# ShuhongChen/panic3d-anime-reconstruction

Hardware: AMD Instinct MI355X
Metric: rendered rays/sec at 512^2 img x 96 samples/ray (higher is better)
Workload: dtype f32

## Files before the change

### panic3d-anime-reconstruction_amd/csrc/p3d_kernels.hip

```cpp
#include <hip/hip_runtime.h>
#include <stddef.h>
#include <stdlib.h>
#include <string.h>

#include <atomic>
#include <type_traits>

#include "p3d_ray_phases.hpp"
#include "p3d_render_plan.hpp"
#include "p3d_cull_band.hpp"
#include "p3d_phase_timing.hpp"

#define P3D_WAVES_PER_WG 4
#define P3D_WG (64 * P3D_WAVES_PER_WG)

__global__ __launch_bounds__(256) void k_planes_to_nhwc(const float* __restrict__ src, float* __restrict__ dst, int HW) {
    __shared__ float tile[32][65];
    const int p0 = blockIdx.x * 64;
    const size_t img = (size_t)blockIdx.y * 32 * HW;
    {
        int px = threadIdx.x & 63, c0 = threadIdx.x >> 6;
#pragma unroll
        for (int k = 0; k < 8; ++k) {
            int c = c0 + 4 * k;
// ... 210 lines not shown
    if (tile >= p.ntiles) return;
    P3D_PHASE(P3D_PH_WEIGHTS);
    float* wl = lds + (FAST ? P3D_LDS_FAST_FLOATS : P3D_LDS_MLP_FLOATS) + 4 + (size_t)wave * p.lds_rows * 32;
    const int Sc = p.Sc, Sf = P3D_NF_EXACT(NF) ? NF : p.Sf, S = Sc + Sf;
    const P3dRayCtx cx = p3d_ray_setup(p, p3d_render_tile_ray(p, tile, j), Sc, Sf);
    const bool active = cx.active;
    const size_t ray = cx.ray;
    const float ox = cx.ox, oy = cx.oy, oz = cx.oz, dx = cx.dx, dy = cx.dy, dz = cx.dz;
    constexpr bool early = EARLY;
    int ndec = 0;

    float* tcA = wl;
    float* wcA = TCG ? wl : tcA + Sc * 32;
    float* tfA = (NF > 0) ? wcA : wcA + Sc * 32;
    uint32_t* mkA = (uint32_t*)(wl + (size_t)(p.lds_rows - ((Sc + 31) >> 5)) * 32);
    const int nmw = (S + 31) >> 5;
    uint32_t* knA = TCG ? (uint32_t*)(wl + (size_t)(Sc > Sf ? Sc : Sf) * 32) : mkA - (size_t)2 * nmw * 32;
    uint32_t* slA = knA + (size_t)nmw * 32;
    const P3dSpacing sp = TCG ? p3d_spacing_fixed(p.ray_start, p.ray_end, p.depth_delta, Sc) : p3d_spacing_of(p, ray, Sc);
    auto tc_raw = [&](int i) -> float { return p3d_stratified_fixed(i, Sc, cx.jitter(i), sp); };
    auto tc_of = [&](int i) -> float { if constexpr (TCG) return tc_raw(i); else return tcA[i * 32 + j]; };
    bool wave_unsorted = false;
    bool bad_order = false;
    bool wave_bad = false;
    auto tc_sorted = [&](int i) -> float { return p3d_coarse_rank(tc_raw, i, Sc, wave_unsorted, wave_bad); };
    uint32_t mw0 = 0u, mw1 = 0u, mw2 = 0u;
    uint32_t fw0 = 0u, fw1 = 0u, fw2 = 0u;
    const bool dump = DUMP && active && h == 0;

    bool unsorted = false;
    float tcmin = __builtin_inff(), tcmax = -__builtin_inff();
    if constexpr (!TCG) {
        float prev = -__builtin_inff();
        for (int i0 = 0; i0 < Sc; i0 += 8) {
            float jv[8];
#pragma unroll
            for (int q = 0; q < 8; ++q) jv[q] = cx.jitter(i0 + q < Sc ? i0 + q : Sc - 1);
#pragma unroll
            for (int q = 0; q < 8; ++q) {
                const int i = i0 + q;
                if (i < Sc) {
                    const float t = p3d_stratified_depth(i, Sc, jv[q], sp);
                    tcA[i * 32 + j] = t;
                    unsorted |= (t < prev);
                    prev = t;
                    tcmin = __builtin_fminf(tcmin, t);
                    tcmax = __builtin_fmaxf(tcmax, t);
                    if constexpr (DUMP) if (dump && p.dumps.depths_coarse) p.dumps.depths_coarse[ray * Sc + i] = t;
                }
            }
        }
    }
    P3D_PHASE(P3D_PH_STRAT);
    float tmin = __builtin_inff(), tmax = -__builtin_inff();
    if (Sf > 0) {
        MarchState st = p3d_march_start();
        uint32_t mword = 0;
        if constexpr (TCG) {
            float prev = -__builtin_inff(), pmax = -__builtin_inff();
            for (int i0 = 0; i0 < Sc; i0 += 8) {
                float jv[8];
#pragma unroll
                for (int q = 0; q < 8; ++q) jv[q] = cx.jitter(i0 + q < Sc ? i0 + q : Sc - 1);
#pragma unroll
                for (int q = 0; q < 8; ++q) {
                    const int i = i0 + q;
                    if (i >= Sc) break;
                    const float t = p3d_stratified_fixed(i, Sc, jv[q], sp);
                    unsorted |= (t < prev);
                    bad_order |= (t < pmax);
                    pmax = __builtin_fmaxf(pmax, prev);
                    prev = t;
                    tcmin = __builtin_fminf(tcmin, t);
                    tcmax = __builtin_fmaxf(tcmax, t);
                    const float px = ox + t * dx, py = oy + t * dy, pz = oz + t * dz;
                    float sigma = P3D_SIGMA_MASKED;
                    const bool cropped = cx.cropped(px, pz);
                    const bool live = !(cropped || st.Td < 1e-60);
                    const bool skip = __builtin_amdgcn_ballot_w64(live) == 0;
                    if (!skip) {
                        f32x16 dummy;
                        p3d_decode_wave<false, true>(lds, cx.rs, cx.g, cx.cfg, px, py, pz, sigma, dummy, live);
                    }
                    mword |= (cropped || (live && sigma == P3D_SIGMA_MASKED)) ? (1u << (i & 31)) : 0u;
                    if ((i & 31) == 31 || i == Sc - 1) {
                        if ((i >> 5) == 0) mw0 = mword; else if ((i >> 5) == 1) mw1 = mword; else mw2 = mword;
                        mword = 0;
                    }
                    if (i > 0) wcA[(i - 1) * 32 + j] = p3d_march_interval(st, t, sigma).w;
                    st.prev_t = t; st.prev_sigma = sigma;
                    ndec += skip ? 0 : 1;
                }
            }
        } else
        for (int i = 0; i < Sc; ++i) {
            float t = tcA[i * 32 + j];
            float px = ox + t * dx, py = oy + t * dy, pz = oz + t * dz;
            float sigma = P3D_SIGMA_MASKED;
            bool skip = false, live = true, cropped = false;
            if (early) {
                cropped = cx.cropped(px, pz);
                live = !(cropped || st.Td < 1e-60);
                skip = __builtin_amdgcn_ballot_w64(live) == 0;
            }
            if (!skip) {
                f32x16 dummy;
                p3d_decode_wave<false, true>(lds, cx.rs, cx.g, cx.cfg, px, py, pz, sigma, dummy, live);
            }
            if (early) {
                mword |= (cropped || (live && sigma == P3D_SIGMA_MASKED)) ? (1u << (i & 31)) : 0u;
                if ((i & 31) == 31 || i == Sc - 1) { mkA[(i >> 5) * 32 + j] = mword; mword = 0; }
            }
            if constexpr (DUMP) if (dump && p.dumps.sigma_coarse) p.dumps.sigma_coarse[ray * Sc + i] = sigma;
            if (i > 0) {
                float w = p3d_march_interval(st, t, sigma).w;
                wcA[(i - 1) * 32 + j] = w;
                if constexpr (DUMP) if (dump && p.dumps.weights_coarse) p.dumps.weights_coarse[ray * (Sc - 1) + i - 1] = w;
            }
            st.prev_t = t; st.prev_sigma = sigma;
            if constexpr (!DUMP) ndec += skip ? 0 : 1;
        }
        P3D_PHASE(P3D_PH_COARSE);
        const int Ns = Sc - 3;
        p3d_pdf_to_cdf<32>(wcA, Ns, j);
        P3D_PHASE(P3D_PH_CDF);
        constexpr int DB = P3D_DRAW_BATCH;
        auto dump_draw = [&](bool mine, int i, float v, int k) {
            if constexpr (DUMP) {
                if (mine && p.dumps.depths_fine) p.dumps.depths_fine[ray * Sf + i] = v;
                if (mine && p.dumps.inds) p.dumps.inds[ray * Sf + i] = k;
            }
        };
        if constexpr (P3D_NF_EXACT(NF)) {
            constexpr int H = NF / 2;
            static_assert(H % DB == 0, "whole batches of draws per half");
            const int d0 = h * H;
            float tf[H];
#pragma unroll
            for (int i = 0; i < H; ++i) tf[i] = cx.u(d0 + i);
#pragma unroll
            for (int i0 = 0; i0 < H; i0 += DB) {
                float ub[DB], vb[DB];
                int kb[DB];
#pragma unroll
                for (int q = 0; q < DB; ++q) ub[q] = tf[i0 + q];
                p3d_inverse_cdf<DB, 32>(wcA, tc_of, Ns, j, ub, vb, kb);
#pragma unroll
                for (int q = 0; q < DB; ++q) {
                    tf[i0 + q] = vb[q];
                    dump_draw(active, d0 + i0 + q, vb[q], kb[q]);
                }
            }
            P3D_PHASE(P3D_PH_DRAWS);
// ... 40 lines not shown
            P3D_PHASE(P3D_PH_DRAWS);
            p3d_sort_network<NF>(tf);
#pragma unroll
            for (int i = 0; i < NF; ++i)
                if (i < Sf) {
                    tfA[i * 32 + j] = tf[i];
                    if constexpr (TCG) {
                        const uint32_t b = cx.cropped_at(tf[i]) ? (1u << (i & 31)) : 0u;
                        if (i < 32) fw0 |= b; else if (i < 64) fw1 |= b; else fw2 |= b;
                    }
                }
        } else {
            for (int i0 = 0; i0 < Sf; i0 += DB) {
                float ub[DB], vb[DB];
                int kb[DB];
#pragma unroll
                for (int q = 0; q < DB; ++q) ub[q] = cx.u(i0 + q < Sf ? i0 + q : Sf - 1);
                p3d_inverse_cdf<DB, 32>(wcA, tc_of, Ns, j, ub, vb, kb);
#pragma unroll
                for (int q = 0; q < DB; ++q) {
                    if (i0 + q < Sf) {
                        tfA[(i0 + q) * 32 + j] = vb[q];
                        dump_draw(dump, i0 + q, vb[q], kb[q]);
                    }
                }
            }
            P3D_PHASE(P3D_PH_DRAWS);
            p3d_lds_insertion_sort(tfA, Sf, j);
        }
        P3D_PHASE(P3D_PH_SORT);
        if constexpr (TCG) {
            wave_unsorted = __builtin_amdgcn_ballot_w64(unsorted) != 0;
            wave_bad = __builtin_amdgcn_ballot_w64(bad_order) != 0;
            if (wave_unsorted) { mw0 = 0u; mw1 = 0u; mw2 = 0u; }
        } else
        if (__builtin_amdgcn_ballot_w64(unsorted) != 0) {
            p3d_lds_insertion_sort(tcA, Sc, j);
            if (early) {
                for (int i = 0; i < ((Sc + 31) >> 5); ++i) mkA[i * 32 + j] = 0u;
            }
        }
    }
    MarchState st = p3d_march_start();
    P3dAccum acc;
    f32x16 prev_rgb = 0.0f;
    {
        int ci = 0, fi = 0;
        float ta = TCG ? 0.0f : tcA[j], tb = (Sf > 0) ? tfA[j] : __builtin_inff();
        tmin = __builtin_fminf(tcmin, tb);
        tmax = __builtin_fmaxf(tcmax, (Sf > 0) ? tfA[(Sf - 1) * 32 + j] : -__builtin_inff());
        bool prev_skipped = false, first = true, done = false;
        int m = 0;
        auto advance = [&](bool take_c) {
            ci += take_c ? 1 : 0;
            fi += take_c ? 0 : 1;
            const int cq = ci < Sc ? ci : Sc - 1, fq = fi < Sf ? fi : (Sf > 0 ? Sf - 1 : 0);
            const float nv = (take_c ? tcA : tfA)[(take_c ? cq : fq) * 32 + j];
            ta = take_c ? nv : ta;
            tb = take_c ? tb : nv;
        };
        float tcn = 0.0f;
        if constexpr (TCG) {
            p3d_merge_bits_ranks(
                tc_sorted, [&](int k) { return tfA[k * 32 + j]; },
                [&](int i, float t) {
                    const uint32_t mwv = (i < 32) ? mw0 : (i < 64 ? mw1 : mw2);
                    return cx.cropped_at(t) || ((mwv >> (i & 31)) & 1u);
                },
                [&](int w, uint32_t kw, uint32_t sw) { knA[w * 32 + j] = kw; slA[w * 32 + j] = sw; }, fw0, fw1, fw2, Sc, Sf, h);
            tcn = tc_sorted(0);
        } else
        if constexpr (EARLY) {
            for (int w = 0; w < nmw; ++w) { knA[w * 32 + j] = 0u; slA[w * 32 + j] = 0u; }
            __builtin_amdgcn_fence(__ATOMIC_ACQ_REL, "wavefront");
            p3d_merge_bits_half(
                [&](bool c, int i) { return (c ? tcA : tfA)[i * 32 + j]; },
                [&](bool c, int i, float t) {
                    bool known = cx.cropped_at(t);
                    if (c && Sf > 0) known = known || ((mkA[(i >> 5) * 32 + j] >> (i & 31)) & 1u);
                    return known;
                },
                [&](int w, uint32_t kw, uint32_t sw) { atomicOr(&knA[w * 32 + j], kw); atomicOr(&slA[w * 32 + j], sw); },
                Sc, Sf, h);
            __builtin_amdgcn_fence(__ATOMIC_ACQ_REL, "wavefront");
            ci = 0;
        }
        P3D_PHASE(P3D_PH_MERGE);
        for (int it = 0;; ++it) {
            bool take_c, known = false;
            float t;
            if constexpr (!EARLY) {
                if (it >= S) break;
                take_c = (ci < Sc) && (fi >= Sf || ta <= tb);
                t = take_c ? ta : tb;
                advance(take_c);
            } else {
                if (!done && (m >= S || st.Td < (FAST ? P3D_FAST_TD_CUT : 1e-60))) done = true;
                if (!done && (first || st.prev_sigma <= 602.0f)) {
                    bool any = false, last_c = false;
                    while (m < S) {
                        const int sh = m & 31, left = (32 - sh < S - m) ? 32 - sh : S - m;
                        const uint32_t kw = knA[(m >> 5) * 32 + j] >> sh, sw = slA[(m >> 5) * 32 + j] >> sh;
                        int run = (~kw != 0u) ? __builtin_ctz(~kw) : 32;
                        run = run < left ? run : left;
                        if (run > 0) {
                            const uint32_t inrun = run >= 32 ? 0xffffffffu : ((1u << run) - 1u);
                            ci += __builtin_popcount(sw & inrun);
                            last_c = (sw >> (run - 1)) & 1u;
                            any = true;
                            m += run;
                        }
                        if (run < left) break;
                    }
// ... 604 lines not shown
                            int force_sigmoid, float* out_sigma, float* out_rgb, void* stream) {
    if (!feats || !w0 || !b0 || !w1 || !b1 || !out_sigma || !out_rgb || N <= 0 || M <= 0) return P3D_E_ARG;
    if ((((uintptr_t)feats | (uintptr_t)out_rgb) & 15) != 0) return P3D_E_RANGE;
    DecodeFeatParams p;
    p.feats = feats; p.w0 = w0; p.b0 = b0; p.w1 = w1; p.b1 = b1; p.out_sigma = out_sigma; p.out_rgb = out_rgb;
    p.M = M; p.tiles_per_img = (M + 31) / 32; p.ntiles = p.tiles_per_img * N;
    memset(&p.cfg, 0, sizeof(p.cfg));
    p.cfg.flags = force_sigmoid ? P3D_FLAG_FORCE_SIGMOID : 0;
    const size_t lds_bytes = (size_t)(P3D_LDS_MLP_FLOATS + 4) * 4;
    long long blocks = (p.ntiles + P3D_WAVES_PER_WG - 1) / P3D_WAVES_PER_WG;
    if (blocks > 256 * 8) blocks = 256 * 8;
    hipError_t e = p3d_ensure_dynamic_lds(k_decode_features, lds_bytes);
    if (e != hipSuccess) return (int)e;
    hipLaunchKernelGGL(k_decode_features, dim3((unsigned)blocks), dim3(P3D_WG), lds_bytes, (hipStream_t)stream, p);
    return p3d_check_launch();
}

size_t p3d_render_workspace_bytes(int N, int64_t R, int Sc, int Sf) {
    (void)R; (void)Sc; (void)Sf;
    return p3d_render_plan_workspace_bytes(N);
}

#ifdef P3D_PHASE_TIMING
int p3d_phase_read(unsigned long long* out, int n, int reset) {
    unsigned long long v[P3D_PH_N];
    if (hipDeviceSynchronize() != hipSuccess || hipMemcpyFromSymbol(v, HIP_SYMBOL(g_p3d_phase), sizeof(v)) != hipSuccess) return -1;
    for (int q = 0; q < n && q < P3D_PH_N; ++q) out[q] = v[q];
    if (reset) {
        memset(v, 0, sizeof(v));
        if (hipMemcpyToSymbol(HIP_SYMBOL(g_p3d_phase), v, sizeof(v)) != hipSuccess) return -1;
    }
    return P3D_PH_N;
}
#endif
int p3d_render_plan_info(int N, int64_t R, int ray_tile_w, const p3d_opts* opts, int has_dumps, int has_ray_limits, int64_t* out, int cap) {
    if (!opts) return P3D_E_ARG;
    const RenderPlan pl = p3d_render_plan(N, R, ray_tile_w, *opts, has_dumps != 0, has_ray_limits != 0);
    if (pl.err) return pl.err;
    if (!out || cap < 6) return P3D_E_ARG;
    const int64_t info[6] = {pl.slots, pl.ntiles, pl.decode_steps_full, pl.grid, pl.block, (int64_t)pl.lds_bytes};
    for (int i = 0; i < 6; ++i) out[i] = info[i];
    return P3D_OK;
}

int p3d_render_f32(const float* planes, int N, int H, int W, const float* rays_o, const float* rays_d, int64_t R,
                   int ray_tile_w, const float* jitter, const float* u, const float* w0, const float* b0,
                   const float* w1, const float* b1, const p3d_opts* opts, float* out_feat, float* out_depth,
                   float* out_wsum, float* out_xyz, void* workspace, size_t workspace_bytes, const p3d_dumps* dumps,
                   void* stream) {
    return p3d_render_limits_f32(planes, N, H, W, rays_o, rays_d, R, ray_tile_w, jitter, u, w0, b0, w1, b1, nullptr, nullptr, opts,
                                 out_feat, out_depth, out_wsum, out_xyz, workspace, workspace_bytes, dumps, stream);
}

static int render_impl(const float* planes, int N, int H, int W, const float* rays_o, const float* rays_d, int64_t R,
                       int ray_tile_w, const float* jitter, const float* u, int rng, uint64_t seed, const float* w0, const float* b0,
                       const float* w1, const float* b1, const float* ray_start, const float* ray_end, const p3d_opts* opts,
                       float* out_feat, float* out_depth, float* out_wsum, float* out_xyz, void* workspace,
                       size_t workspace_bytes, const p3d_dumps* dumps, void* stream);

int p3d_render_limits_f32(const float* planes, int N, int H, int W, const float* rays_o, const float* rays_d, int64_t R,
                          int ray_tile_w, const float* jitter, const float* u, const float* w0, const float* b0,
                          const float* w1, const float* b1, const float* ray_start, const float* ray_end, const p3d_opts* opts,
                          float* out_feat, float* out_depth, float* out_wsum, float* out_xyz, void* workspace,
                          size_t workspace_bytes, const p3d_dumps* dumps, void* stream) {
    return render_impl(planes, N, H, W, rays_o, rays_d, R, ray_tile_w, jitter, u, 0, 0, w0, b0, w1, b1, ray_start, ray_end, opts, out_feat,
                       out_depth, out_wsum, out_xyz, workspace, workspace_bytes, dumps, stream);
// ... 9 lines not shown

static int render_impl(const float* planes, int N, int H, int W, const float* rays_o, const float* rays_d, int64_t R,
                       int ray_tile_w, const float* jitter, const float* u, int rng, uint64_t seed, const float* w0, const float* b0,
                       const float* w1, const float* b1, const float* ray_start, const float* ray_end, const p3d_opts* opts,
                       float* out_feat, float* out_depth, float* out_wsum, float* out_xyz, void* workspace,
                       size_t workspace_bytes, const p3d_dumps* dumps, void* stream) {
    if ((ray_start == nullptr) != (ray_end == nullptr)) return P3D_E_ARG;
    if (!planes || !rays_o || !rays_d || (!jitter && !rng) || !w0 || !b0 || !w1 || !b1 || !opts || !out_feat || !out_depth ||
        !out_wsum || !out_xyz || !workspace || N <= 0 || R <= 0)
        return P3D_E_ARG;
    const int Sc = opts->Sc, Sf = opts->Sf;
    if (Sc < 4 || Sc > P3D_MAX_S || Sf < 0 || Sf > P3D_MAX_S) return P3D_E_RANGE;
    if (Sf > 0 && !u && !rng) return P3D_E_ARG;
    if (H <= 0 || W <= 0 || (long long)H * W * 128 * 3 >= 0x7ffffff0LL) return P3D_E_RANGE;
    if (workspace_bytes < p3d_render_plan_workspace_bytes(N)) return P3D_E_WORKSPACE;
    const RenderPlan pl = p3d_render_plan(N, R, ray_tile_w, *opts, dumps != nullptr, ray_start != nullptr);
    if (pl.err) return pl.err;
    hipStream_t st = (hipStream_t)stream;
    RenderParams p;
    p.planes = planes; p.rays_o = rays_o; p.rays_d = rays_d; p.jitter = jitter; p.u = u;
    p.rng = rng; p.seed_lo = (uint32_t)seed; p.seed_hi = (uint32_t)(seed >> 32);
    p.w0 = w0; p.b0 = b0; p.w1 = w1; p.b1 = b1;
    p.out_feat = out_feat; p.out_depth = out_depth; p.out_wsum = out_wsum; p.out_xyz = out_xyz;
    p.gminmax = (uint32_t*)workspace;
    p.per_view_clamp = (opts->flags & P3D_FLAG_PER_VIEW_CLAMP) ? 1 : 0;
    if (dumps) p.dumps = *dumps; else memset(&p.dumps, 0, sizeof(p.dumps));
    p.R = R; p.H = H; p.W = W; p.Sc = Sc; p.Sf = Sf;
    p.ray_start = opts->ray_start; p.ray_end = opts->ray_end; p.depth_delta = opts->depth_delta;
    p.ray_start_arr = ray_start; p.ray_end_arr = ray_end;
    p.disparity = (opts->flags & P3D_FLAG_DISPARITY) ? 1 : 0;
    p.white_back = (opts->flags & P3D_FLAG_WHITE_BACK) ? 1 : 0;
    p.cfg = make_cfg(opts);
    p.tile_w = pl.tile_w; p.tiles_x = pl.tiles_x; p.tiles_per_img = pl.tiles_per_img; p.ntiles = pl.ntiles;
    p.lds_rows = pl.lds_rows; p.swz = pl.swz; p.blocked = pl.blocked;
    hipLaunchKernelGGL(k_minmax_init, dim3((unsigned)((N + 255) / 256)), dim3(256), 0, st, p.gminmax, p.per_view_clamp ? N : 0);
    auto launch = [&](void (*kernel)(RenderParams)) {
        hipError_t e = p3d_ensure_dynamic_lds(kernel, pl.lds_bytes);
        if (e != hipSuccess) return (int)e;
        hipLaunchKernelGGL(kernel, dim3(pl.grid), dim3(pl.block), pl.lds_bytes, st, p);
        return p3d_check_launch();
    };
    const int rc = p3d_with_nf(pl.nf, [&](auto nfc) {
        constexpr int NF = decltype(nfc)::value;
        if constexpr (NF == 48 || NF == 96)
            if (pl.kernel == RenderKernel::SLOTS4_WO) return launch(k_render_slots<4, NF, true, true>);
        auto mode = [&](auto fc) {
            constexpr bool F = decltype(fc)::value;
            switch (pl.kernel) {
            case RenderKernel::DUMP: return launch(k_render<NF, true, F, false>);
            case RenderKernel::PLAIN: return launch(k_render<NF, false, F, false>);
            case RenderKernel::EARLY_TCG: return launch(k_render<NF, false, F, true>);
            case RenderKernel::EARLY: return launch(k_render<NF, false, F, true, false>);
            case RenderKernel::SLOTS2: return launch(k_render_slots<2, NF, F>);
            default: return launch(k_render_slots<4, NF, F>);
            }
        };
        return pl.fast ? mode(std::true_type()) : mode(std::false_type());
    });
    if (rc) return rc;
    long long NR = (long long)N * R;
    hipLaunchKernelGGL(k_render_finish, dim3((unsigned)((NR + 255) / 256)), dim3(256), 0, st, out_depth, NR, p.gminmax,
                       dumps ? dumps->tminmax : nullptr, p.per_view_clamp ? (long long)R : 0LL);
    return p3d_check_launch();
}

int p3d_sample_stratified_f32(float ray_start, float ray_end, float depth_delta, int S, const float* jitter, int64_t NR,
                              float* out, void* stream) {
// ... 68 lines not shown
```

### panic3d-anime-reconstruction_amd/csrc/p3d_ray_phases.hpp

```cpp
#pragma once
#include "p3d_decode.hpp"
#include "p3d_importance.hpp"

struct RenderParams {
    const float* planes;
    const float *rays_o, *rays_d;
    const float* jitter;
    const float* u;
    const float *w0, *b0, *w1, *b1;
    float *out_feat, *out_depth, *out_wsum, *out_xyz;
    uint32_t* gminmax;
    int per_view_clamp;
    p3d_dumps dumps;
    long long R;
    long long tiles_per_img, ntiles;
    int tile_w;
    int tiles_x;
    int H, W;
    int Sc, Sf;
    float ray_start, ray_end, depth_delta;
    const float *ray_start_arr, *ray_end_arr;
    int disparity;
    int white_back;
    int lds_rows;
    int rng;
    uint32_t seed_lo, seed_hi;
    int swz;
    int blocked;
    P3dDecodeCfg cfg;
};

P3D_DEV long long p3d_render_wave_tile(const RenderParams& p, int wave) {
    long long nblk = gridDim.x, b = blockIdx.x;
    const long long swz = p.swz;
    long long full = (nblk / (8 * swz)) * (8 * swz);
    long long bs = b;
    if (b < full) {
        long long slot = b >> 3, x = b & 7;
        const long long g = slot / swz, xr = p.blocked ? ((x + g) & 7) : x;
        bs = g * (8 * swz) + xr * swz + (slot % swz);
    }
    const int nwaves = blockDim.x >> 6;
    return bs * nwaves + wave;
}

struct P3dTileRay { long long n, r; };

P3D_DEV P3dTileRay p3d_render_tile_ray(const RenderParams& p, long long tile, int j) {
    P3dTileRay o;
    o.n = tile / p.tiles_per_img;
    const long long tl = tile - o.n * p.tiles_per_img;
    if (p.tile_w > 0) {
        long long ty = tl / p.tiles_x, tx = tl - ty * p.tiles_x;
        if (p.blocked) {
            const long long st = tl >> 8;
            const int q = (int)(tl & 255), SX = p.tiles_x >> 4;
            tx = (st % SX) * 16 + (q & 15);
            ty = (st / SX) * 16 + (q >> 4);
        }
        const int lx = (j & 1) | ((j >> 1) & 6), ly = ((j >> 1) & 1) | ((j >> 3) & 2);
        o.r = (ty * 4 + ly) * p.tile_w + tx * 8 + lx;
    } else {
        o.r = tl * 32 + j;
    }
    return o;
}

template <int RPW>
P3D_DEV P3dTileRay p3d_slots_tile_ray(const RenderParams& p, long long tile, int jr) {
    P3dTileRay o;
    o.n = tile / p.tiles_per_img;
    const long long tl = tile - o.n * p.tiles_per_img;
    if (p.tile_w > 0) {
        long long ty = tl / p.tiles_x, tx = tl - ty * p.tiles_x;
        const int lx = (jr & 1) | ((jr >> 1) & 2), ly = ((jr >> 1) & 1) | ((jr >> 2) & 2);
        o.r = (ty * (RPW / 4) + ly) * p.tile_w + tx * 4 + lx;
    } else {
        o.r = tl * RPW + jr;
    }
    return o;
}

P3D_DEV uint32_t p3d_fmix32(uint32_t h) {
    h ^= h >> 16; h *= 0x85EBCA6Bu; h ^= h >> 13; h *= 0xC2B2AE35u; h ^= h >> 16;
    return h;
}
P3D_DEV float p3d_draw(uint32_t seed_lo, uint32_t seed_hi, uint32_t stream, size_t ray, int idx) {
    uint32_t h = p3d_fmix32(seed_lo ^ ((uint32_t)ray * 0x9E3779B1u));
    h = p3d_fmix32(h ^ seed_hi ^ ((uint32_t)((unsigned long long)ray >> 32) * 0x7FEB352Du) ^ (((uint32_t)idx * 2u + stream) * 0x846CA68Bu));
    return (float)(h >> 8) * 0x1p-24f;
}

P3D_DEV bool p3d_crop_xz(const bool& f_crop, const float& crop_limit, float px, float pz) {
    return f_crop && (__builtin_fabsf(px) > crop_limit || __builtin_fabsf(pz) > crop_limit);
}

typedef decltype(__builtin_amdgcn_make_buffer_rsrc((void*)nullptr, (short)0, 0, 0)) p3d_rsrc_t;

struct P3dRayCtx {
    bool active;
    size_t ray;
    unsigned nlo;
    P3dPlaneGeom g;
    p3d_rsrc_t rs;
    P3dDecodeCfg cfg;
    bool f_crop;
    float ox, oy, oz, dx, dy, dz;
    int rng;
    uint32_t seed_lo, seed_hi;
    const float *jit, *uu;
    P3D_DEV float jitter(int i) const { return rng ? p3d_draw(seed_lo, seed_hi, 0u, ray, i) : jit[i]; }
    P3D_DEV float u(int i) const { return rng ? p3d_draw(seed_lo, seed_hi, 1u, ray, i) : uu[i]; }
    P3D_DEV bool cropped(float px, float pz) const { return p3d_crop_xz(f_crop, cfg.crop_limit, px, pz); }
    P3D_DEV bool cropped_at(float t) const { return cropped(ox + t * dx, oz + t * dz); }
};

P3D_DEV P3dRayCtx p3d_ray_setup(const RenderParams& p, P3dTileRay tr, int Sc, int Sf) {
    P3dRayCtx c;
    c.active = tr.r < p.R;
    const long long rc = c.active ? tr.r : p.R - 1;
    c.ray = (size_t)tr.n * p.R + rc;
    c.g.halfW = 0.5f * (float)p.W; c.g.halfH = 0.5f * (float)p.H; c.g.fW = (float)p.W; c.g.fH = (float)p.H; c.g.W = p.W;
    c.g.plane_bytes = (uint32_t)p.H * (uint32_t)p.W * 128u;
    c.nlo = __builtin_amdgcn_readfirstlane((unsigned)tr.n);
    const float* pbase = p.planes + ((p.cfg.flags & P3D_FLAG_SHARED_PLANES) ? (size_t)0 : (size_t)c.nlo * 3 * (c.g.plane_bytes / 4));
    c.rs = __builtin_amdgcn_make_buffer_rsrc((void*)pbase, 0, 3 * c.g.plane_bytes, 0x00020000);
    c.cfg = p.cfg;
    c.f_crop = (c.cfg.flags & P3D_FLAG_CROP) != 0;
    c.ox = p.rays_o[c.ray * 3]; c.oy = p.rays_o[c.ray * 3 + 1]; c.oz = p.rays_o[c.ray * 3 + 2];
    c.dx = p.rays_d[c.ray * 3]; c.dy = p.rays_d[c.ray * 3 + 1]; c.dz = p.rays_d[c.ray * 3 + 2];
    c.rng = p.rng; c.seed_lo = p.seed_lo; c.seed_hi = p.seed_hi;
    c.jit = p.jitter + c.ray * Sc;
    c.uu = p.u + c.ray * Sf;
    return c;
}

struct P3dSpacing {
    float ray_start, ray_end, depth_delta, step;
    bool limits;
    float rs, span, rdelta;
    bool disparity;
};
P3D_DEV P3dSpacing p3d_spacing_fixed(float ray_start, float ray_end, float depth_delta, int Sc) {
    return {ray_start, ray_end, depth_delta, (ray_end - ray_start) / (float)(Sc - 1), false, 0.0f, 0.0f, 0.0f, false};
}
P3D_DEV P3dSpacing p3d_spacing_of(const RenderParams& p, size_t ray, int Sc) {
    P3dSpacing s = p3d_spacing_fixed(p.ray_start, p.ray_end, p.depth_delta, Sc);
// ... 18 lines not shown
        const float l01 = (i < Sc / 2) ? p3d_fma(s01, (float)i, 0.0f) : p3d_fma(-s01, (float)(Sc - 1 - i), 1.0f);
        const float dd = l01 + jv * s.depth_delta;
        const float ta_ = s.ray_start * (1.0f - dd), tb_ = s.ray_end * dd;
        t = 1.0f / (ta_ + tb_);
    }
    return t;
}

struct MarchState {
    double Td;
    float W, D;
    float prev_t, prev_sigma;
};
P3D_DEV MarchState p3d_march_start(float t0 = 0.0f, float sigma0 = 0.0f) { return {1.0, 0.0f, 0.0f, t0, sigma0}; }
struct P3dInterval { float w, tm, alpha, T; };
P3D_DEV P3dInterval p3d_march_interval(MarchState& st, float t, float sigma) {
    P3dInterval iv;
    float dl = t - st.prev_t;
    float sm = (st.prev_sigma + sigma) * 0.5f;
    iv.tm = (st.prev_t + t) * 0.5f;
    float rho = p3d_softplus(sm - 1.0f);
    float dd = rho * dl;
    iv.alpha = 1.0f - p3d_exp(-dd);
    iv.T = (float)st.Td;
    iv.w = iv.alpha * iv.T;
    st.Td = st.Td * (double)((1.0f - iv.alpha) + 1e-10f);
    return iv;
}
P3D_DEV void p3d_march_accumulate(MarchState& st, const P3dInterval& iv) {
    st.W = st.W + iv.w;
    st.D = p3d_fma(iv.w, iv.tm, st.D);
}

P3D_DEV float p3d_pdf_bin(float wa, float wb, float wc) {
    float m1 = __builtin_fmaxf(wa, wb), m2 = __builtin_fmaxf(wb, wc);
    return ((m1 + m2) * 0.5f + 0.01f) + 1e-5f;
}
P3D_DEV float p3d_cdf_step(double& acc, float v, float fsum) {
    float pdf = v / fsum;
    acc += (double)pdf;
    return (float)acc;
}
template <int RS>
P3D_DEV void p3d_pdf_to_cdf(float* A, int Ns, int j) {
    double sum = 0.0;
    float wa = A[0 * RS + j], wb = A[1 * RS + j];
    for (int jj = 0; jj < Ns; ++jj) {
        float wc = A[(jj + 2) * RS + j];
        float v = p3d_pdf_bin(wa, wb, wc);
        sum += (double)v;
        A[(jj + 1) * RS + j] = v;
        wa = wb; wb = wc;
    }
    float fsum = (float)sum;
    double acc = 0.0;
    A[j] = 0.0f;
    for (int jj = 0; jj < Ns; ++jj) A[(jj + 1) * RS + j] = p3d_cdf_step(acc, A[(jj + 1) * RS + j], fsum);
}

template <int B, int RS, typename TCF>
P3D_DEV void p3d_inverse_cdf(const float* cdfA, TCF tc, int Ns, int j, const float (&ui)[B], float (&out)[B], int (&k_out)[B]) {
    const int n = Ns + 1;
    int pos[B];
#pragma unroll
    for (int q = 0; q < B; ++q) pos[q] = 0;
#pragma unroll
// ... 136 lines not shown
```

### panic3d-anime-reconstruction_amd/csrc/p3d_phase_timing.hpp

```cpp
#pragma once

#ifdef P3D_PHASE_TIMING
enum P3dPhase {
    P3D_PH_WEIGHTS = 0,
    P3D_PH_STRAT,
    P3D_PH_COARSE,
    P3D_PH_CDF,
    P3D_PH_DRAWS,
    P3D_PH_SORT,
    P3D_PH_MERGE,
    P3D_PH_SELECT,
    P3D_PH_DECODE,
    P3D_PH_MARCH,
    P3D_PH_OUT,
    P3D_PH_WAVES,
    P3D_PH_LIFE,
    P3D_PH_N
};
__device__ unsigned long long g_p3d_phase[P3D_PH_N];

struct P3dPhaseClock {
    unsigned long long first, last, acc[P3D_PH_N];
    __device__ __forceinline__ static unsigned long long now() {
        unsigned long long t;
        __builtin_amdgcn_sched_barrier(0);
        asm volatile("s_memtime %0\n\ts_waitcnt lgkmcnt(0)" : "=s"(t) :: "memory");
        __builtin_amdgcn_sched_barrier(0);
        return t;
    }
    __device__ __forceinline__ void start() {
#pragma unroll
        for (int q = 0; q < P3D_PH_N; ++q) acc[q] = 0ull;
        first = last = now();
    }
    __device__ __forceinline__ void mark(int slot) {
        const unsigned long long t = now();
        acc[slot] += t - last;
        last = t;
    }
    __device__ __forceinline__ void flush() {
        acc[P3D_PH_WAVES] = 1ull;
        acc[P3D_PH_LIFE] = last - first;
        if ((threadIdx.x & 63) == 0) {
#pragma unroll
            for (int q = 0; q < P3D_PH_N; ++q) atomicAdd(&g_p3d_phase[q], acc[q]);
        }
    }
};
#define P3D_PHASE_START() P3dPhaseClock p3d_phase_clock; p3d_phase_clock.start()
#define P3D_PHASE(slot) p3d_phase_clock.mark(slot)
#define P3D_PHASE_FLUSH() p3d_phase_clock.flush()
#else
#define P3D_PHASE_START() ((void)0)
#define P3D_PHASE(slot) ((void)0)
#define P3D_PHASE_FLUSH() ((void)0)
#endif
```

### panic3d-anime-reconstruction_amd/csrc/p3d_render_plan.hpp

```cpp
#pragma once
#include <stddef.h>
#include <stdint.h>

#include "../../include/panic3d_hip.h"
#include "p3d_lds_layout.hpp"

#define P3D_RENDER_WAVES 4
#define P3D_RENDER_LDS_CU (160 * 1024)

constexpr bool p3d_render_tcg(int NF, bool DUMP, bool EARLY) { return NF == 96 && EARLY && !DUMP; }
constexpr int p3d_render_occ(int NF, bool TCG) { return (NF >= 96 && !TCG) ? 1 : 2; }
constexpr int p3d_render_slots_occ(int SLOTS, bool FAST) { return (SLOTS == 4 && FAST) ? 2 : 1; }

enum class RenderKernel {
    DUMP,
    PLAIN,
    EARLY,
    EARLY_TCG,
    SLOTS2,
    SLOTS4,
    SLOTS4_WO,
};

struct RenderPlan {
    int err;
    RenderKernel kernel;
    int nf;
    bool fast;
    int slots;
    int rays_per_wave;
    int tile_w, tiles_x;
    long long tiles_per_img, ntiles;
    int lds_rows;
    int nwaves;
    unsigned grid, block;
    size_t lds_bytes;
    int swz, blocked;
    long long decode_steps_full;
};

static inline size_t p3d_render_plan_workspace_bytes(int N) {
    return 256 + (size_t)(N > 0 ? N : 0) * 8;
}

static inline RenderPlan p3d_render_plan(int N, int64_t R, int ray_tile_w, const p3d_opts& o, bool has_dumps, bool has_ray_limits) {
    RenderPlan pl = {};
    const int Sc = o.Sc, Sf = o.Sf, flags = o.flags;
    const bool disparity = (flags & P3D_FLAG_DISPARITY) != 0;
    if (N <= 0 || R <= 0) pl.err = P3D_E_ARG;
    else if (Sc < 4 || Sc > P3D_MAX_S || Sf < 0 || Sf > P3D_MAX_S) pl.err = P3D_E_RANGE;
    else if (disparity && has_ray_limits) pl.err = P3D_E_RANGE;
    if (pl.err) return pl;

    pl.nf = (Sf == 48) ? 48 : (Sf == 96 && Sc <= 96) ? 96 : (Sf <= 64 ? 64 : 0);
    pl.fast = (flags & P3D_FLAG_FAST_COLOR) != 0 && Sf > 0;
    const bool tiled = ray_tile_w > 0 && R % ray_tile_w == 0 && ray_tile_w % 8 == 0 && (R / ray_tile_w) % 4 == 0;
    const auto tile = [&](int rpw) {
        const int tw = rpw == 32 ? 8 : 4;
        pl.rays_per_wave = rpw;
        pl.tile_w = tiled ? ray_tile_w : 0;
        pl.tiles_x = tiled ? ray_tile_w / tw : 0;
        pl.tiles_per_img = tiled ? (long long)pl.tiles_x * (R / ray_tile_w / (rpw / tw)) : (R + rpw - 1) / rpw;
        pl.ntiles = pl.tiles_per_img * N;
    };
    tile(32);

    const bool small = !has_dumps && !(flags & P3D_FLAG_NO_PAIR) && pl.ntiles <= 512;
    const bool quad = small && !(flags & P3D_FLAG_PAIR16) &&
                      ((flags & P3D_FLAG_QUAD8) || (long long)N * R <= 8192 || (pl.fast && (pl.nf == 96 || pl.nf == 48)));
    const bool tcg = pl.nf == 96 && !has_dumps && !small && !(flags & P3D_FLAG_NO_EARLY_OUT) && !has_ray_limits && !disparity;
// ... 5 lines not shown

    int nw = P3D_RENDER_WAVES;
    if (small) {
        pl.slots = quad ? 4 : 2;
        tile(32 / pl.slots);
        const bool wo = quad && pl.fast && (flags & P3D_FLAG_WEIGHTS_ONLY) != 0 && (pl.nf == 48 || pl.nf == 96);
        pl.kernel = wo ? RenderKernel::SLOTS4_WO : quad ? RenderKernel::SLOTS4 : RenderKernel::SLOTS2;
        const size_t wgs = quad ? 2 : 1;
        while (nw > 1 && wgs * lds(nw) > P3D_RENDER_LDS_CU) nw >>= 1;
    } else {
        pl.slots = 1;
        pl.kernel = has_dumps ? RenderKernel::DUMP : (flags & P3D_FLAG_NO_EARLY_OUT) ? RenderKernel::PLAIN
                                                   : tcg ? RenderKernel::EARLY_TCG : RenderKernel::EARLY;
        while (nw > 1 && pl.ntiles / nw < 2 * 256) nw >>= 1;
        if (nw == P3D_RENDER_WAVES) {
            const int occ = p3d_render_occ(pl.nf, tcg);
            int best = 0, best_waves = 0;
            for (int w = P3D_RENDER_WAVES; w >= 1; w >>= 1) {
                if (lds(w) > P3D_RENDER_LDS_CU) continue;
                const int fit = (int)(P3D_RENDER_LDS_CU / lds(w)) * w;
                const int waves = fit > 4 * occ ? 4 * occ / w * w : fit;
                if (waves > best_waves) { best_waves = waves; best = w; }
            }
            if (best == 0) { pl.err = P3D_E_RANGE; return pl; }
            nw = best;
        }
        while (nw > 1 && lds(nw) > P3D_RENDER_LDS_CU) nw >>= 1;
        pl.swz = 16;
        const long long tiles_y = tiled ? pl.tiles_per_img / pl.tiles_x : 0;
        if (tiled && pl.tiles_x % 16 == 0 && tiles_y % 16 == 0 && 256 % nw == 0 && (pl.ntiles / 256) % 8 == 0) {
            pl.blocked = 1;
            pl.swz = 256 / nw;
        }
    }
    if (lds(nw) > P3D_RENDER_LDS_CU) { pl.err = P3D_E_RANGE; return pl; }
    pl.nwaves = nw;
    pl.lds_bytes = lds(nw);
    pl.grid = (unsigned)((pl.ntiles + nw - 1) / nw);
    pl.block = 64 * nw;
    const auto steps = [&](int S) { return (long long)((S + pl.slots - 1) / pl.slots); };
    pl.decode_steps_full = pl.ntiles * (Sf > 0 ? steps(Sc) + steps(Sc + Sf) : steps(Sc));
    return pl;
}
```

Measured before the change: 91.09 million.

## Skip coarse march intervals for wave-wide dead samples and precompute crop masks

Crop bits for coarse samples are now computed during stratification (or after sorting) and stored in the mask words, so the coarse march and the merge no longer recompute crop tests. A new P3dCoarseSkip helper lets the coarse loop bypass the march-interval arithmetic entirely when no lane in the wave is live and the previous sample was not 'hot', writing zero weights and resuming from the stale previous depth later. This removes exp/softplus/double work for empty regions, at the cost of extra state tracking and a heuristic threshold (sigma <= 602) that assumes masked-sigma intervals contribute exactly zero.

```diff
diff --git a/panic3d-anime-reconstruction_amd/csrc/p3d_kernels.hip b/panic3d-anime-reconstruction_amd/csrc/p3d_kernels.hip
--- a/panic3d-anime-reconstruction_amd/csrc/p3d_kernels.hip
+++ b/panic3d-anime-reconstruction_amd/csrc/p3d_kernels.hip
@@ -266,6 +266,7 @@
     float tcmin = __builtin_inff(), tcmax = -__builtin_inff();
     if constexpr (!TCG) {
         float prev = -__builtin_inff();
+        uint32_t cword = 0u;
         for (int i0 = 0; i0 < Sc; i0 += 8) {
             float jv[8];
 #pragma unroll
@@ -281,7 +282,12 @@
                     tcmin = __builtin_fminf(tcmin, t);
                     tcmax = __builtin_fmaxf(tcmax, t);
                     if constexpr (DUMP) if (dump && p.dumps.depths_coarse) p.dumps.depths_coarse[ray * Sc + i] = t;
+                    if constexpr (EARLY) cword |= cx.cropped_at_flat(t) ? (1u << (i & 31)) : 0u;
                 }
+            }
+            if constexpr (EARLY) {
+                mkA[(i0 >> 5) * 32 + j] = cword;
+                if (((i0 + 8) & 31) == 0) cword = 0u;
             }
         }
     }
@@ -290,6 +296,7 @@
     if (Sf > 0) {
         MarchState st = p3d_march_start();
         uint32_t mword = 0;
+        P3dCoarseSkip cs;
         if constexpr (TCG) {
             float prev = -__builtin_inff(), pmax = -__builtin_inff();
             for (int i0 = 0; i0 < Sc; i0 += 8) {
@@ -304,46 +311,57 @@
                     unsorted |= (t < prev);
                     bad_order |= (t < pmax);
                     pmax = __builtin_fmaxf(pmax, prev);
+                    const float tprev = prev;
                     prev = t;
                     tcmin = __builtin_fminf(tcmin, t);
                     tcmax = __builtin_fmaxf(tcmax, t);
-                    const float px = ox + t * dx, py = oy + t * dy, pz = oz + t * dz;
-                    float sigma = P3D_SIGMA_MASKED;
-                    const bool cropped = cx.cropped(px, pz);
-                    const bool live = !(cropped || st.Td < 1e-60);
+                    const bool cropped = cx.cropped_at_flat(t);
+                    mword |= cropped ? (1u << (i & 31)) : 0u;
+                    const bool live = !(cropped || cs.dead);
                     const bool skip = __builtin_amdgcn_ballot_w64(live) == 0;
-                    if (!skip) {
-                        f32x16 dummy;
-                        p3d_decode_wave<false, true>(lds, cx.rs, cx.g, cx.cfg, px, py, pz, sigma, dummy, live);
+                    if (cs.identity(skip)) {
+                        if (i > 0) wcA[(i - 1) * 32 + j] = 0.0f;
+                    } else {
+                        cs.resume(st, [&] { return tprev; });
+                        const float px = ox + t * dx, py = oy + t * dy, pz = oz + t * dz;
+                        float sigma = P3D_SIGMA_MASKED;
+                        if (!skip) {
+                            f32x16 dummy;
+                            p3d_decode_wave<false, true>(lds, cx.rs, cx.g, cx.cfg, px, py, pz, sigma, dummy, live);
+                            mword |= (live && sigma == P3D_SIGMA_MASKED) ? (1u << (i & 31)) : 0u;
+                            ndec += 1;
+                        }
+                        if (i > 0) wcA[(i - 1) * 32 + j] = p3d_march_interval(st, t, sigma).w;
+                        st.prev_t = t; st.prev_sigma = sigma;
+                        cs.marched(st, !skip, sigma);
                     }
-                    mword |= (cropped || (live && sigma == P3D_SIGMA_MASKED)) ? (1u << (i & 31)) : 0u;
                     if ((i & 31) == 31 || i == Sc - 1) {
                         if ((i >> 5) == 0) mw0 = mword; else if ((i >> 5) == 1) mw1 = mword; else mw2 = mword;
                         mword = 0;
                     }
-                    if (i > 0) wcA[(i - 1) * 32 + j] = p3d_march_interval(st, t, sigma).w;
-                    st.prev_t = t; st.prev_sigma = sigma;
-                    ndec += skip ? 0 : 1;
                 }
             }
         } else
         for (int i = 0; i < Sc; ++i) {
+            if (early && (i & 31) == 0) mword = mkA[(i >> 5) * 32 + j];
+            const bool live = !(early && (((mword >> (i & 31)) & 1u) != 0u || cs.dead));
+            const bool skip = early && __builtin_amdgcn_ballot_w64(live) == 0;
+            if (cs.identity(skip)) {
+                if (i > 0) wcA[(i - 1) * 32 + j] = 0.0f;
+                continue;
+            }
+            cs.resume(st, [&] { return tcA[(i - 1) * 32 + j]; });
             float t = tcA[i * 32 + j];
             float px = ox + t * dx, py = oy + t * dy, pz = oz + t * dz;
             float sigma = P3D_SIGMA_MASKED;
-            bool skip = false, live = true, cropped = false;
-            if (early) {
-                cropped = cx.cropped(px, pz);
-                live = !(cropped || st.Td < 1e-60);
-                skip = __builtin_amdgcn_ballot_w64(live) == 0;
-            }
             if (!skip) {
                 f32x16 dummy;
                 p3d_decode_wave<false, true>(lds, cx.rs, cx.g, cx.cfg, px, py, pz, sigma, dummy, live);
-            }
-            if (early) {
-                mword |= (cropped || (live && sigma == P3D_SIGMA_MASKED)) ? (1u << (i & 31)) : 0u;
-                if ((i & 31) == 31 || i == Sc - 1) { mkA[(i >> 5) * 32 + j] = mword; mword = 0; }
+                if (early) {
+                    mword |= (live && sigma == P3D_SIGMA_MASKED) ? (1u << (i & 31)) : 0u;
+                    mkA[(i >> 5) * 32 + j] = mword;
+                }
+                if constexpr (!DUMP) ndec += 1;
             }
             if constexpr (DUMP) if (dump && p.dumps.sigma_coarse) p.dumps.sigma_coarse[ray * Sc + i] = sigma;
             if (i > 0) {
@@ -352,7 +370,7 @@
                 if constexpr (DUMP) if (dump && p.dumps.weights_coarse) p.dumps.weights_coarse[ray * (Sc - 1) + i - 1] = w;
             }
             st.prev_t = t; st.prev_sigma = sigma;
-            if constexpr (!DUMP) ndec += skip ? 0 : 1;
+            if (early) cs.marched(st, !skip, sigma);
         }
         P3D_PHASE(P3D_PH_COARSE);
         const int Ns = Sc - 3;
@@ -459,12 +477,22 @@
         if constexpr (TCG) {
             wave_unsorted = __builtin_amdgcn_ballot_w64(unsorted) != 0;
             wave_bad = __builtin_amdgcn_ballot_w64(bad_order) != 0;
-            if (wave_unsorted) { mw0 = 0u; mw1 = 0u; mw2 = 0u; }
+            if (wave_unsorted) {
+                mw0 = 0u; mw1 = 0u; mw2 = 0u;
+                for (int i = 0; i < Sc; ++i) {
+                    const uint32_t b = cx.cropped_at(tc_sorted(i)) ? (1u << (i & 31)) : 0u;
+                    if (i < 32) mw0 |= b; else if (i < 64) mw1 |= b; else mw2 |= b;
+                }
+            }
         } else
         if (__builtin_amdgcn_ballot_w64(unsorted) != 0) {
             p3d_lds_insertion_sort(tcA, Sc, j);
             if (early) {
-                for (int i = 0; i < ((Sc + 31) >> 5); ++i) mkA[i * 32 + j] = 0u;
+                uint32_t cword = 0u;
+                for (int i = 0; i < Sc; ++i) {
+                    cword |= cx.cropped_at(tcA[i * 32 + j]) ? (1u << (i & 31)) : 0u;
+                    if ((i & 31) == 31 || i == Sc - 1) { mkA[(i >> 5) * 32 + j] = cword; cword = 0u; }
+                }
             }
         }
     }
@@ -490,9 +518,9 @@
         if constexpr (TCG) {
             p3d_merge_bits_ranks(
                 tc_sorted, [&](int k) { return tfA[k * 32 + j]; },
-                [&](int i, float t) {
+                [&](int i, float) {
                     const uint32_t mwv = (i < 32) ? mw0 : (i < 64 ? mw1 : mw2);
-                    return cx.cropped_at(t) || ((mwv >> (i & 31)) & 1u);
+                    return ((mwv >> (i & 31)) & 1u) != 0u;
                 },
                 [&](int w, uint32_t kw, uint32_t sw) { knA[w * 32 + j] = kw; slA[w * 32 + j] = sw; }, fw0, fw1, fw2, Sc, Sf, h);
             tcn = tc_sorted(0);
@@ -503,9 +531,8 @@
             p3d_merge_bits_half(
                 [&](bool c, int i) { return (c ? tcA : tfA)[i * 32 + j]; },
                 [&](bool c, int i, float t) {
-                    bool known = cx.cropped_at(t);
-                    if (c && Sf > 0) known = known || ((mkA[(i >> 5) * 32 + j] >> (i & 31)) & 1u);
-                    return known;
+                    const bool cbit = ((mkA[(c ? i >> 5 : 0) * 32 + j] >> (i & 31)) & 1u) != 0u;
+                    return c ? cbit : cx.cropped_at(t);
                 },
                 [&](int w, uint32_t kw, uint32_t sw) { atomicOr(&knA[w * 32 + j], kw); atomicOr(&slA[w * 32 + j], sw); },
                 Sc, Sf, h);
diff --git a/panic3d-anime-reconstruction_amd/csrc/p3d_ray_phases.hpp b/panic3d-anime-reconstruction_amd/csrc/p3d_ray_phases.hpp
--- a/panic3d-anime-reconstruction_amd/csrc/p3d_ray_phases.hpp
+++ b/panic3d-anime-reconstruction_amd/csrc/p3d_ray_phases.hpp
@@ -113,6 +113,10 @@
     P3D_DEV float u(int i) const { return rng ? p3d_draw(seed_lo, seed_hi, 1u, ray, i) : uu[i]; }
     P3D_DEV bool cropped(float px, float pz) const { return p3d_crop_xz(f_crop, cfg.crop_limit, px, pz); }
     P3D_DEV bool cropped_at(float t) const { return cropped(ox + t * dx, oz + t * dz); }
+    P3D_DEV bool cropped_at_flat(float t) const {
+        const float px = ox + t * dx, pz = oz + t * dz;
+        return f_crop & ((__builtin_fabsf(px) > cfg.crop_limit) | (__builtin_fabsf(pz) > cfg.crop_limit));
+    }
 };
 
 P3D_DEV P3dRayCtx p3d_ray_setup(const RenderParams& p, P3dTileRay tr, int Sc, int Sf) {
@@ -197,6 +201,29 @@
     st.D = p3d_fma(iv.w, iv.tm, st.D);
 }
 
+struct P3dCoarseSkip {
+    bool hot = false;
+    bool stale = false;
+    bool dead = false;
+    P3D_DEV bool identity(bool nolive) {
+        const bool id = nolive && !hot;
+        stale = stale || id;
+        return id;
+    }
+    template <typename TP>
+    P3D_DEV void resume(MarchState& st, TP tprev) {
+        if (stale) {
+            st.prev_t = tprev();
+            st.prev_sigma = P3D_SIGMA_MASKED;
+            stale = false;
+        }
+    }
+    P3D_DEV void marched(const MarchState& st, bool decoded, float sigma) {
+        hot = decoded && __builtin_amdgcn_ballot_w64(!(sigma <= 602.0f)) != 0;
+        dead = st.Td < 1e-60;
+    }
+};
+
 P3D_DEV float p3d_pdf_bin(float wa, float wb, float wc) {
     float m1 = __builtin_fmaxf(wa, wb), m2 = __builtin_fmaxf(wb, wc);
     return ((m1 + m2) * 0.5f + 0.01f) + 1e-5f;
```

New measurement: 91.55 million, median of 6. About the same (+0.5%).

## Assign screen tiles to blocks in small pieces balanced across XCDs

Applied to the files above, without the earlier changes.

Replaces the 16x16 blocked tile swizzle with a piece-based order. Each piece is 2x8 tiles, and pieces are spread over the eight XCDs with a rotation rule that is checked to give every XCD an equal share of the central rows. The intent is to even out per-XCD work, since rays near the image centre are presumably costlier, while keeping neighbouring tiles together for cache reuse of the planes. It also adds per-wave start/end realtime and XCC-id recording to the phase-timing build for profiling. The risk is lower L2 locality than the larger 16x16 blocks, and the mapping only applies when the tile counts divide evenly.

```diff
diff --git a/panic3d-anime-reconstruction_amd/csrc/p3d_kernels.hip b/panic3d-anime-reconstruction_amd/csrc/p3d_kernels.hip
--- a/panic3d-anime-reconstruction_amd/csrc/p3d_kernels.hip
+++ b/panic3d-anime-reconstruction_amd/csrc/p3d_kernels.hip
@@ -1176,6 +1176,18 @@
     }
     return P3D_PH_N;
 }
+int p3d_phase_read_waves(unsigned long long* out, int n) {
+    if (!out || n < 0 || n > P3D_WAVE_RECORDS) return -1;
+    P3dWaveRecord* v = (P3dWaveRecord*)malloc(sizeof(P3dWaveRecord) * (size_t)(n > 0 ? n : 1));
+    if (!v) return -1;
+    const bool ok = hipDeviceSynchronize() == hipSuccess &&
+                    hipMemcpyFromSymbol(v, HIP_SYMBOL(g_p3d_wave), sizeof(P3dWaveRecord) * (size_t)n) == hipSuccess;
+    for (int i = 0; ok && i < n; ++i) {
+        out[4 * i] = v[i].t0; out[4 * i + 1] = v[i].t1; out[4 * i + 2] = v[i].block; out[4 * i + 3] = v[i].xcc;
+    }
+    free(v);
+    return ok ? n : -1;
+}
 #endif
 int p3d_render_plan_info(int N, int64_t R, int ray_tile_w, const p3d_opts* opts, int has_dumps, int has_ray_limits, int64_t* out, int cap) {
     if (!opts) return P3D_E_ARG;
@@ -1251,7 +1263,7 @@
     p.white_back = (opts->flags & P3D_FLAG_WHITE_BACK) ? 1 : 0;
     p.cfg = make_cfg(opts);
     p.tile_w = pl.tile_w; p.tiles_x = pl.tiles_x; p.tiles_per_img = pl.tiles_per_img; p.ntiles = pl.ntiles;
-    p.lds_rows = pl.lds_rows; p.swz = pl.swz; p.blocked = pl.blocked;
+    p.lds_rows = pl.lds_rows; p.order = pl.order;
     hipLaunchKernelGGL(k_minmax_init, dim3((unsigned)((N + 255) / 256)), dim3(256), 0, st, p.gminmax, p.per_view_clamp ? N : 0);
     auto launch = [&](void (*kernel)(RenderParams)) {
         hipError_t e = p3d_ensure_dynamic_lds(kernel, pl.lds_bytes);
diff --git a/panic3d-anime-reconstruction_amd/csrc/p3d_phase_timing.hpp b/panic3d-anime-reconstruction_amd/csrc/p3d_phase_timing.hpp
--- a/panic3d-anime-reconstruction_amd/csrc/p3d_phase_timing.hpp
+++ b/panic3d-anime-reconstruction_amd/csrc/p3d_phase_timing.hpp
@@ -18,9 +18,12 @@
     P3D_PH_N
 };
 __device__ unsigned long long g_p3d_phase[P3D_PH_N];
+#define P3D_WAVE_RECORDS 65536
+struct P3dWaveRecord { unsigned long long t0, t1; unsigned block, xcc; };
+__device__ P3dWaveRecord g_p3d_wave[P3D_WAVE_RECORDS];
 
 struct P3dPhaseClock {
-    unsigned long long first, last, acc[P3D_PH_N];
+    unsigned long long first, last, real0, acc[P3D_PH_N];
     __device__ __forceinline__ static unsigned long long now() {
         unsigned long long t;
         __builtin_amdgcn_sched_barrier(0);
@@ -28,9 +31,17 @@
         __builtin_amdgcn_sched_barrier(0);
         return t;
     }
+    __device__ __forceinline__ static unsigned long long real_now() {
+        unsigned long long t;
+        __builtin_amdgcn_sched_barrier(0);
+        asm volatile("s_memrealtime %0\n\ts_waitcnt lgkmcnt(0)" : "=s"(t) :: "memory");
+        __builtin_amdgcn_sched_barrier(0);
+        return t;
+    }
     __device__ __forceinline__ void start() {
 #pragma unroll
         for (int q = 0; q < P3D_PH_N; ++q) acc[q] = 0ull;
+        real0 = real_now();
         first = last = now();
     }
     __device__ __forceinline__ void mark(int slot) {
@@ -44,6 +55,14 @@
         if ((threadIdx.x & 63) == 0) {
 #pragma unroll
             for (int q = 0; q < P3D_PH_N; ++q) atomicAdd(&g_p3d_phase[q], acc[q]);
+            const unsigned long long slot = (unsigned long long)blockIdx.x * (blockDim.x >> 6) + (threadIdx.x >> 6);
+            if (slot < P3D_WAVE_RECORDS) {
+                unsigned xcc;
+                asm volatile("s_getreg_b32 %0, hwreg(HW_REG_XCC_ID, 0, 4)" : "=s"(xcc));
+                P3dWaveRecord r;
+                r.t0 = real0; r.t1 = real_now(); r.block = blockIdx.x; r.xcc = xcc;
+                g_p3d_wave[slot] = r;
+            }
         }
     }
 };
diff --git a/panic3d-anime-reconstruction_amd/csrc/p3d_ray_phases.hpp b/panic3d-anime-reconstruction_amd/csrc/p3d_ray_phases.hpp
--- a/panic3d-anime-reconstruction_amd/csrc/p3d_ray_phases.hpp
+++ b/panic3d-anime-reconstruction_amd/csrc/p3d_ray_phases.hpp
@@ -1,6 +1,7 @@
 #pragma once
 #include "p3d_decode.hpp"
 #include "p3d_importance.hpp"
+#include "p3d_render_plan.hpp"
 
 struct RenderParams {
     const float* planes;
@@ -25,43 +26,26 @@
     int lds_rows;
     int rng;
     uint32_t seed_lo, seed_hi;
-    int swz;
-    int blocked;
+    P3dTileOrder order;
     P3dDecodeCfg cfg;
 };
 
 P3D_DEV long long p3d_render_wave_tile(const RenderParams& p, int wave) {
-    long long nblk = gridDim.x, b = blockIdx.x;
-    const long long swz = p.swz;
-    long long full = (nblk / (8 * swz)) * (8 * swz);
-    long long bs = b;
-    if (b < full) {
-        long long slot = b >> 3, x = b & 7;
-        const long long g = slot / swz, xr = p.blocked ? ((x + g) & 7) : x;
-        bs = g * (8 * swz) + xr * swz + (slot % swz);
-    }
-    const int nwaves = blockDim.x >> 6;
-    return bs * nwaves + wave;
+    return p3d_tile_of_block(p.order, gridDim.x, blockIdx.x, blockDim.x >> 6, wave, p.tiles_x, p.tiles_per_img);
 }
 
 struct P3dTileRay { long long n, r; };
 
 P3D_DEV P3dTileRay p3d_render_tile_ray(const RenderParams& p, long long tile, int j) {
     P3dTileRay o;
-    o.n = tile / p.tiles_per_img;
-    const long long tl = tile - o.n * p.tiles_per_img;
     if (p.tile_w > 0) {
-        long long ty = tl / p.tiles_x, tx = tl - ty * p.tiles_x;
-        if (p.blocked) {
-            const long long st = tl >> 8;
-            const int q = (int)(tl & 255), SX = p.tiles_x >> 4;
-            tx = (st % SX) * 16 + (q & 15);
-            ty = (st / SX) * 16 + (q >> 4);
-        }
+        const P3dTileXY t = p3d_tile_screen(p.order, tile, p.tiles_x, p.tiles_per_img);
+        o.n = t.n;
         const int lx = (j & 1) | ((j >> 1) & 6), ly = ((j >> 1) & 1) | ((j >> 3) & 2);
-        o.r = (ty * 4 + ly) * p.tile_w + tx * 8 + lx;
+        o.r = (t.ty * 4 + ly) * p.tile_w + t.tx * 8 + lx;
     } else {
-        o.r = tl * 32 + j;
+        o.n = tile / p.tiles_per_img;
+        o.r = (tile - o.n * p.tiles_per_img) * 32 + j;
     }
     return o;
 }
diff --git a/panic3d-anime-reconstruction_amd/csrc/p3d_render_plan.hpp b/panic3d-anime-reconstruction_amd/csrc/p3d_render_plan.hpp
--- a/panic3d-anime-reconstruction_amd/csrc/p3d_render_plan.hpp
+++ b/panic3d-anime-reconstruction_amd/csrc/p3d_render_plan.hpp
@@ -11,6 +11,84 @@
 constexpr bool p3d_render_tcg(int NF, bool DUMP, bool EARLY) { return NF == 96 && EARLY && !DUMP; }
 constexpr int p3d_render_occ(int NF, bool TCG) { return (NF >= 96 && !TCG) ? 1 : 2; }
 constexpr int p3d_render_slots_occ(int SLOTS, bool FAST) { return (SLOTS == 4 && FAST) ? 2 : 1; }
+
+#if defined(__HIPCC__)
+#define P3D_HD __host__ __device__ __forceinline__
+#else
+#define P3D_HD static inline
+#endif
+
+struct P3dTileOrder {
+    int swz;
+    int blocked;
+    int pieces;
+    int pw, ph, xa, xs;
+};
+
+#ifndef P3D_PIECE_W
+#define P3D_PIECE_W 2
+#define P3D_PIECE_H 8
+#define P3D_XCD_RULE_A 1
+#define P3D_XCD_RULE_S 0
+#endif
+
+static inline bool p3d_piece_order(P3dTileOrder& t, long long tiles_x, long long tiles_y, int nw, int pw, int ph, int xa, int xs) {
+    if (pw <= 0 || ph <= 0 || tiles_x <= 0 || tiles_x % pw || tiles_y % ph || (pw * ph) % nw || (tiles_y / ph) % 8) return false;
+    const long long PC = tiles_x / pw, PR = tiles_y / ph;
+    long long inner[8] = {0, 0, 0, 0, 0, 0, 0, 0};
+    for (long long r = PR / 4; r < PR - PR / 4; ++r)
+        for (long long c = 0; c < PC; ++c) ++inner[(xa * c + r + xs * (r / 8)) & 7];
+    for (int x = 0; x < 8; ++x)
+        if (2 * inner[x] != PC * PR / 8) return false;
+    t.pieces = 1;
+    t.swz = pw * ph / nw;
+    t.pw = pw; t.ph = ph; t.xa = xa; t.xs = xs;
+    return true;
+}
+
+P3D_HD long long p3d_tile_of_block(const P3dTileOrder& t, long long nblk, long long b, int nwaves, int wave, int tiles_x,
+                                   long long tiles_per_img) {
+    const long long swz = t.swz;
+    long long bs = b;
+    if (t.pieces) {
+        const int x = (int)(b & 7), PC = tiles_x / t.pw, per_img = (int)(tiles_per_img / (t.pw * t.ph)), per_xcd = per_img >> 3;
+        const int per_col = per_xcd / PC;
+        const long long slot = b >> 3, k = slot / swz;
+        const int n = (int)(k / per_xcd), kk = (int)(k - (long long)n * per_xcd), c = kk / per_col, j = kk - c * per_col;
+        const int r = ((x - t.xa * c - t.xs * j) & 7) + 8 * j;
+        bs = ((long long)n * per_img + (long long)r * PC + c) * swz + (slot - k * swz);
+    } else {
+        const long long full = (nblk / (8 * swz)) * (8 * swz);
+        if (b < full) {
+            const long long slot = b >> 3, x = b & 7;
+            const long long g = slot / swz, xr = t.blocked ? ((x + g) & 7) : x;
+            bs = g * (8 * swz) + xr * swz + (slot % swz);
+        }
+    }
+    return bs * nwaves + wave;
+}
+
+struct P3dTileXY { long long n, tx, ty; };
+
+P3D_HD P3dTileXY p3d_tile_screen(const P3dTileOrder& t, long long tile, int tiles_x, long long tiles_per_img) {
+    P3dTileXY o;
+    o.n = tile / tiles_per_img;
+    const long long tl = tile - o.n * tiles_per_img;
+    o.ty = tl / tiles_x;
+    o.tx = tl - o.ty * tiles_x;
+    if (t.pieces) {
+        const long long pc = tl / (t.pw * t.ph);
+        const int q = (int)(tl - pc * (t.pw * t.ph)), PC = tiles_x / t.pw;
+        o.tx = (pc % PC) * t.pw + (q % t.pw);
+        o.ty = (pc / PC) * t.ph + (q / t.pw);
+    } else if (t.blocked) {
+        const long long st = tl >> 8;
+        const int q = (int)(tl & 255), SX = tiles_x >> 4;
+        o.tx = (st % SX) * 16 + (q & 15);
+        o.ty = (st / SX) * 16 + (q >> 4);
+    }
+    return o;
+}
 
 enum class RenderKernel {
     DUMP,
@@ -36,6 +114,7 @@
     unsigned grid, block;
     size_t lds_bytes;
     int swz, blocked;
+    P3dTileOrder order;
     long long decode_steps_full;
 };
 
@@ -107,6 +186,11 @@
             pl.blocked = 1;
             pl.swz = 256 / nw;
         }
+        pl.order.swz = pl.swz;
+        pl.order.blocked = pl.blocked;
+#ifndef P3D_TILE_ORDER_PARENT
+        if (pl.blocked) p3d_piece_order(pl.order, pl.tiles_x, tiles_y, nw, P3D_PIECE_W, P3D_PIECE_H, P3D_XCD_RULE_A, P3D_XCD_RULE_S);
+#endif
     }
     if (lds(nw) > P3D_RENDER_LDS_CU) { pl.err = P3D_E_RANGE; return pl; }
     pl.nwaves = nw;
```

Result: faster. 91.02 million before, 94.48 million after (median of 6 runs) (+3.8%).
